# terminusdb-labs/parallel-hnsw

Hardware: AMD Instinct MI355X
Metric: queries/sec at recall@10≥0.95 on 1M×768 f32 (higher is better)
Workload: dtype f32

## Files before the change

### parallel_hnsw_amd/csrc/api.hip

```cpp
#include <hip/hip_runtime.h>

#include <algorithm>
#include <atomic>
#include <cmath>
#include <cstdarg>
#include <cstdio>
#include <cstring>
#include <new>
#include <stdexcept>
#include <vector>

#include "exact_slices.h"
#include "phnsw_internal.h"

static thread_local std::string g_err;

void ph_set_error(const char *fmt, ...) {
  char buf[1024];
  va_list ap;
  va_start(ap, fmt);
  vsnprintf(buf, sizeof(buf), fmt, ap);
  va_end(ap);
  g_err = buf;
}
// ... 763 lines not shown
    if (!rc && c.first_node + nq <= B.n_nodes) rc = ph_layer_range_order(B, c.first_node, (uint32_t)nq, &a.order);
    if (rc) return rc;
  }
  const bool split = (ph_store_f32(ix->store) || ph_store_converted(ix->store)) && !a.order && !knn_mode && !out_stride && !out_index && first_big < a.n_layers &&
                     nq >= two_launch_min() &&
                     !getenv("PHNSW_NO_LOCALITY");
  if (split) {
    g_two_launch_count++;
    rc = ph_workspace_order_ensure(ws, a.nq);
    for (uint32_t l = first_big; l < a.n_layers && !rc; l++)
      rc = ph_layer_anchor_pos(ix->store, mix->layers[l - 1]);
    if (rc) return rc;
    if (a.collect_k) {
      const size_t need = (size_t)nq * a.ef * 4u;
      if (ws.park_ids_bytes < need) {
        if (ws.park_ids) PH_HIP(hipFree(ws.park_ids));
        ws.park_ids = nullptr, ws.park_ids_bytes = 0;
        PH_HIP(hipMalloc(&ws.park_ids, need));
        ws.park_ids_bytes = need;
      }
      if (ws.park_d_bytes < need) {
        if (ws.park_d) PH_HIP(hipFree(ws.park_d));
        ws.park_d = nullptr, ws.park_d_bytes = 0;
        PH_HIP(hipMalloc(&ws.park_d, need));
        ws.park_d_bytes = need;
      }
      a.out_ids = ws.park_ids;
      a.out_d = ws.park_d;
    }
  }
  const uint32_t *table_pos = nullptr;
  const char *const table_order_env = getenv("PHNSW_TABLE_ORDER");
  if (T && !split && !a.order && !knn_mode && !out_stride && !out_index && !c.hint && !c.out_hit && !a.filter && !a.label_of && !a.attr_of && !a.pair_of &&
      !a.collect_k && nq >= PH_TABLE_ORDER_MIN && !getenv("PHNSW_NO_LOCALITY") && !(table_order_env && table_order_env[0] == '0')) {
    PhLayerHost &TL = mix->layers[T - 1];
    rc = ph_layer_anchor_pos(ix->store, TL);
    if (!rc && TL.pos) rc = ph_workspace_order_ensure(ws, a.nq);
    if (rc) return rc;
    table_pos = TL.pos;
  }
  rc = attach_probes(mix, c, a);
  if (rc) return rc;
  rc = ph_search_begin(ws, stream);
  if (rc) return rc;
  bool kept_table = false;
  if (c.hint && T && !split) {
    rc = ph_build_table_prepare(mix, ws, a, *c.hint, T, stream, &kept_table);
    if (rc) return rc;
  }
  const uint64_t tmax = (T && !kept_table) ? ph_tiny_max_positions(ix, a.n_layers, a.ef) : 0;
  const uint64_t chunk = (tmax && nq > tmax) ? tmax : nq;
  for (uint64_t c0 = 0; c0 < nq; c0 += chunk) {
    PhSearchArgs b = a;
    const uint64_t cnt = std::min<uint64_t>(chunk, nq - c0);
    const bool last_chunk = c0 + cnt == nq;
    b.nq = (uint32_t)cnt;
    if (b.order) {
      b.order += c0;
    } else if (c0) {
      const uint32_t ostride = out_stride ? out_stride : b.ef;
      if (b.queries) b.queries += c0 * c.ldq;
      if (b.qids) b.qids += c0;
      if (b.exclude) b.exclude += c0;
      if (b.filter) b.filter += c0 * b.filter_stride;
      if (b.label_want) b.label_want += c0;
      if (b.range_lo) b.range_lo += c0, b.range_hi += c0;
      if (b.pair_want) b.pair_want += c0;
      if (b.pair_lo) b.pair_lo += c0, b.pair_hi += c0;
      if (b.set_first) b.set_first += c0;
      if (b.out_ids) b.out_ids += c0 * ostride, b.out_d += c0 * ostride;
      if (b.collect_k) b.collect_ids += c0 * b.collect_k, b.collect_d += c0 * b.collect_k;
      b.out_len += c0;
      if (b.out_stats) b.out_stats += 2 * c0;
      b.status += c0;
      if (b.out_hit) b.out_hit += c0;
      b.first_node += (uint32_t)c0;
    }
    ws.n_chunks = (uint32_t)(c0 / chunk) + 1;
    PH_HIP(hipEventRecord(ws.evc, stream));
    if (c0) PH_HIP(hipMemsetAsync(ws.dtotals, 0, sizeof(unsigned long long) * 3 * PH_MAX_DISPATCH, stream));
    if (!kept_table) {
      rc = ph_tiny_prepare(ix, ws, b, T, stream);
      if (!rc && table_pos && b.tiny_layers == T) {
        rc = ph_tiny_table_order(ws, b, table_pos, ix->store->n_anchors, stream);
        if (!rc && b.table_by_query) g_table_order_count++;
      }
      if (rc) return rc;
    }
    ws.d_tiny = b.tiny_layers != 0;
    PH_HIP(hipEventRecord(ws.evd[0], stream));
    if (!split) {
      b.launch_totals = ws.dtotals;
      b.launch_tab = ws.dtotals + 2 * PH_MAX_DISPATCH;
      rc = ph_search_launch(ix, ws, b, stream, last_chunk);
      if (rc) return rc;
      PH_HIP(hipEventRecord(ws.evd[1], stream));
      ws.n_dispatch = 1;
      ws.d_lo[0] = knn_mode ? b.n_layers - 1 : 0;
      ws.d_hi[0] = b.n_layers;
      continue;
    }
    const uint32_t Td = b.tiny_layers;
    const bool dense_first = Td && Td < b.n_layers && b.nq >= PH_DENSE_SPLIT_MIN && !getenv("PHNSW_NO_DENSE_SPLIT");
    if (dense_first) b.dense_flag = ws.tiny_member + b.tiny_n;
    uint32_t di = 0;
    uint32_t *const out_hit_final = b.out_hit;
    const uint32_t first_hi = dense_first ? Td : first_big;
    for (uint32_t lo = 0, hi = first_hi; lo < b.n_layers; lo = hi, hi = (lo == Td && dense_first && first_big > Td) ? first_big : hi + 1) {
      PhSearchArgs p = b;
      const bool last = hi == b.n_layers;
      p.layer_lo = lo;
      p.layer_hi = hi;
      if (lo) p.tiny_layers = 0;
      if (dense_first) {
        p.dense_only = lo == 0 ? 1u : 0u;
        p.after_dense = lo == Td ? Td : 0u;
      }
      if (!last && p.collect_k) {
        p.collect_k = p.collect_flags = 0u;
        p.filter = nullptr, p.filter_stride = 0u;
        p.label_of = p.label_want = nullptr;
      }
      p.order = lo ? ws.oorder : nullptr;
      p.out_hit = last ? out_hit_final : nullptr;
      p.out_key = last ? nullptr : ws.okey;
      p.key_pos = last ? nullptr : ix->layers[hi - 1].pos;
      p.launch_totals = ws.dtotals + 2 * di;
      p.launch_tab = ws.dtotals + 2 * PH_MAX_DISPATCH + di;
      rc = ph_search_launch(ix, ws, p, stream, last && last_chunk);
      if (!rc && !last) rc = ph_workspace_order_sort(ws, b.nq, stream);
      if (rc) return rc;
      PH_HIP(hipEventRecord(ws.evd[1 + di], stream));
      ws.d_lo[di] = lo;
      ws.d_hi[di] = hi;
      ws.n_dispatch = ++di;
    }
  }
  return 0;
}

static int check_device_call(const char *call, const phnsw_index *ix, const PhSearchCall &c) {
  int rc = ph_check_sp(ix, c.sp);
  if (rc) return rc;
  if ((!c.queries && !c.qids) || !c.out_ids || !c.out_d || !c.out_len || !c.status || c.nq > 0xFFFFFFFFull ||
      (c.queries && (c.ldq < ix->store->ld || (c.ldq % 4) || ((uintptr_t)c.queries % 16)))) {
    ph_set_error("%s: invalid argument (queries need ldq >= store ld, multiple of 4, 16-byte base)", call);
    return PHNSW_E_INVALID;
  }
  return 0;
}

static PhSearchCall device_call(const float *queries_dev, uint32_t ldq, const uint32_t *qids_dev, uint64_t nq,
                                const phnsw_search_params *sp, uint32_t upto_layers, const uint32_t *exclude_dev,
                                uint32_t *out_ids_dev, float *out_d_dev, uint32_t *out_len_dev, uint32_t *out_stats_dev,
                                uint32_t *status_dev, void *stream) {
  PhSearchCall c = {};
  c.queries = queries_dev, c.ldq = ldq, c.qids = qids_dev, c.exclude = exclude_dev, c.nq = nq;
  c.sp = sp, c.upto = upto_layers;
  c.out_ids = out_ids_dev, c.out_d = out_d_dev, c.out_len = out_len_dev, c.status = status_dev;
  c.out_stats = out_stats_dev;
  c.stream = (hipStream_t)stream;
  return c;
}

extern "C" int phnsw_search_batch_device(const phnsw_index *ix, const float *queries_dev, uint32_t ldq,
                                         const uint32_t *qids_dev, uint64_t nq, const phnsw_search_params *sp,
                                         uint32_t upto_layers, const uint32_t *exclude_dev, uint32_t *out_ids_dev,
// ... 591 lines not shown
```

### parallel_hnsw_amd/csrc/bruteforce.hip

```cpp
#include <hip/hip_runtime.h>

#include <algorithm>
#include <cstring>
#include <vector>

#include "phnsw_device.h"

typedef float f32x16 __attribute__((ext_vector_type(16)));

#define BF_TM 128
#define BF_TN 128
#define BF_TK 32
#define BF_LD 132

__global__ __launch_bounds__(256) void ph_gemm_nt_mfma_kernel(const float *__restrict__ Q, uint32_t ldq, uint32_t nq,
                                                              const float *__restrict__ B, uint32_t ldb, uint32_t nb,
                                                              uint32_t K, float *__restrict__ C, uint64_t ldc) {
  __shared__ float Qs[BF_TK][BF_LD];
  __shared__ float Bs[BF_TK][BF_LD];
  const uint32_t t = threadIdx.x, lane = t & 63, w = t >> 6;
  const uint32_t wm = w >> 1, wn = w & 1;
  const uint32_t q0 = blockIdx.y * BF_TM, b0 = blockIdx.x * BF_TN;
  f32x16 acc[2][2];
#pragma unroll
// ... 273 lines not shown
}

__global__ __launch_bounds__(256) void ph_anchor_mean_kernel(const float *__restrict__ rows, uint64_t row_stride, uint32_t ld,
                                                             const uint32_t *__restrict__ start,
                                                             const uint32_t *__restrict__ members, uint32_t A,
                                                             const float *__restrict__ old, float *__restrict__ out) {
  __shared__ float wsum[4];
  const uint32_t a = blockIdx.x, t = threadIdx.x;
  if (a >= A) return;
  const uint32_t first = start[a], cnt = start[a + 1u] - first;
  float ss = 0.f;
  for (uint32_t j = t; j < ld; j += 256u) {
    float acc = 0.f;
    for (uint32_t i = 0; i < cnt; i++) acc += rows[(uint64_t)members[first + i] * row_stride + j];
    out[(uint64_t)a * ld + j] = acc;
    ss += acc * acc;
  }
#pragma unroll
  for (int sft = 32; sft >= 1; sft >>= 1) ss += __shfl_xor(ss, sft);
  if ((t & 63u) == 0) wsum[t >> 6] = ss;
  __syncthreads();
  const float norm = sqrtf(((wsum[0] + wsum[1]) + wsum[2]) + wsum[3]);
  const bool keep = !(norm > 0.f) || !(norm < PH_FMAX);
  for (uint32_t j = t; j < ld; j += 256u)
    out[(uint64_t)a * ld + j] = keep ? old[(uint64_t)a * ld + j] : out[(uint64_t)a * ld + j] / norm;
}

#define PH_CELL_SAMPLE 262144u

static int ph_refine_anchors(const phnsw_store *s, uint32_t A, const float *raw, float *refined) {
  const uint32_t ld = s->ld, m = (uint32_t)std::min<uint64_t>(s->n, PH_CELL_SAMPLE);
  const uint64_t step = s->n / m;
  const uint32_t QC = 65536;
  float *samp = nullptr, *scores = nullptr;
  uint32_t *cell = nullptr, *start = nullptr, *members = nullptr, *ids = nullptr;
  const float *base = s->rows;
  uint64_t row_stride = step * ld;
  int rc = 0;
  hipError_t e = hipMalloc(&scores, (size_t)std::min(QC, m) * A * 4);
  if (e == hipSuccess) e = hipMalloc(&cell, (size_t)m * 4);
  if (e == hipSuccess) e = hipMalloc(&start, ((size_t)A + 1u) * 4);
  if (e == hipSuccess) e = hipMalloc(&members, (size_t)m * 4);
  if (e == hipSuccess && (ph_store_converted(s) || row_stride > 0xFFFFFFFCull)) {
    std::vector<uint32_t> h(m);
    for (uint32_t i = 0; i < m; i++) h[i] = (uint32_t)(i * step);
    e = hipMalloc(&samp, (size_t)m * ld * 4);
    if (e == hipSuccess) e = hipMalloc(&ids, (size_t)m * 4);
    if (e == hipSuccess) e = hipMemcpy(ids, h.data(), (size_t)m * 4, hipMemcpyHostToDevice);
    if (e == hipSuccess) {
      if (ph_store_converted(s))
        rc = ph_converted_gather_rows(s, ids, 0, m, samp);
      else
        hipLaunchKernelGGL(ph_gather_rows_f32_kernel, dim3((m + 3) / 4), dim3(256), 0, 0, s->rows, ld, ids, 1u, m, samp);
    }
    base = samp;
    row_stride = ld;
  }
  if (e == hipSuccess && !rc) {
    for (uint32_t at = 0; at < m; at += QC) {
      const uint32_t cnt = std::min(QC, m - at);
      dim3 grid((A + BF_TN - 1) / BF_TN, (cnt + BF_TM - 1) / BF_TM);
      hipLaunchKernelGGL(ph_gemm_nt_mfma_kernel, grid, dim3(256), 0, 0, base + (uint64_t)at * row_stride, (uint32_t)row_stride,
                         cnt, raw, ld, A, ld, scores, (uint64_t)A);
      hipLaunchKernelGGL(ph_argmax_rows_kernel, dim3(std::min<uint32_t>(cnt, 256u * 16u)), dim3(64), 0, 0, scores, (uint64_t)A,
                         A, cnt, cell + at);
    }
    rc = ph_cell_order_device(cell, m, A, start, members, 0);
    if (!rc) {
      hipLaunchKernelGGL(ph_anchor_mean_kernel, dim3(A), dim3(256), 0, 0, base, row_stride, ld, start, members, A, raw, refined);
      e = hipGetLastError();
      if (e == hipSuccess) e = hipDeviceSynchronize();
    }
  }
  if (e != hipSuccess) rc = ph_hip_fail(e, "store cells (anchor means)", __FILE__, __LINE__);
  if (samp) hipFree(samp);
  if (ids) hipFree(ids);
  if (scores) hipFree(scores);
  if (cell) hipFree(cell);
  if (start) hipFree(start);
  if (members) hipFree(members);
  return rc;
}

static int ph_store_anchors(phnsw_store *s) {
  if (s->anchors) return 0;
  uint32_t amax = 4096u;
  if (const char *e = getenv("PHNSW_ANCHORS")) amax = atoi(e) >= 64 ? (uint32_t)atoi(e) : amax;
  const uint32_t A = (uint32_t)std::min<uint64_t>(amax, std::max<uint64_t>(s->n / 16u, 1u)), ld = s->ld;
  const uint64_t stride = s->n / A;
  const char *const cells_env = getenv("PHNSW_CELLS");
  const bool cells_raw = cells_env && !strcmp(cells_env, "raw");
  float *anchors = nullptr, *gram = nullptr;
  uint32_t *rank = nullptr, *ids = nullptr;
  std::vector<uint32_t> h(A);
  for (uint32_t a = 0; a < A; a++) h[a] = (uint32_t)(a * stride);
  hipError_t e = hipMalloc(&anchors, (size_t)A * ld * 4);
  if (e == hipSuccess) e = hipMalloc(&gram, (size_t)A * A * 4);
  if (e == hipSuccess) e = hipMalloc(&rank, (size_t)A * 4);
  if (e == hipSuccess) e = hipMalloc(&ids, (size_t)A * 4);
  if (e == hipSuccess) e = hipMemcpy(ids, h.data(), (size_t)A * 4, hipMemcpyHostToDevice);
  if (e == hipSuccess) {
    if (ph_store_converted(s))
      (void)ph_converted_gather_rows(s, ids, 0, A, anchors);
    else
      hipLaunchKernelGGL(ph_gather_rows_f32_kernel, dim3((A + 3) / 4), dim3(256), 0, 0, s->rows, ld, ids, 1u, A, anchors);
    if (!cells_raw) {
      float *refined = nullptr;
      e = hipMalloc(&refined, (size_t)A * ld * 4);
      if (e == hipSuccess && ph_refine_anchors(s, A, anchors, refined)) e = hipErrorUnknown;
      if (e == hipSuccess) std::swap(anchors, refined);
      if (refined) hipFree(refined);
    }
  }
  if (e == hipSuccess) {
    dim3 grid((A + BF_TN - 1) / BF_TN, (A + BF_TM - 1) / BF_TM);
    hipLaunchKernelGGL(ph_gemm_nt_mfma_kernel, grid, dim3(256), 0, 0, anchors, ld, A, anchors, ld, A, ld, gram, (uint64_t)A);
    hipLaunchKernelGGL(ph_anchor_chain_kernel, dim3(1), dim3(1024), (A + 32) * 4, 0, gram, A, rank);
    e = hipGetLastError();
    if (e == hipSuccess) e = hipDeviceSynchronize();
  }
  if (gram) hipFree(gram);
  if (ids) hipFree(ids);
  if (e != hipSuccess) {
    if (anchors) hipFree(anchors);
    if (rank) hipFree(rank);
    return ph_hip_fail(e, "store cells (anchors)", __FILE__, __LINE__);
  }
  s->anchors = anchors;
  s->anchor_rank = rank;
  s->n_anchors = A;
  s->cells_raw = cells_raw;
  return 0;
}

void ph_store_anchors_free(phnsw_store *s) {
  if (s->anchors) hipFree(s->anchors);
  if (s->anchor_rank) hipFree(s->anchor_rank);
  s->anchors = nullptr;
  s->anchor_rank = nullptr;
}

bool ph_layer_wants_cells(const phnsw_store *s, uint32_t n_nodes) {
  return n_nodes >= PH_POS_MIN && (ph_store_f32(s) || ph_store_converted(s)) && s->n >= 65536 && s->metric != PHNSW_METRIC_L2 && !getenv("PHNSW_NO_LOCALITY");
}

int ph_layer_cells_range(const phnsw_store *cs, const PhLayerHost &L, uint32_t first, uint32_t count, uint32_t *out_pos) {
  phnsw_store *s = const_cast<phnsw_store *>(cs);
  if (count == 0) return 0;
  int rc = ph_store_anchors(s);
  if (rc) return rc;
  const uint32_t A = s->n_anchors, ld = s->ld;
  const uint32_t QC = 65536;
  float *qrows = nullptr, *scores = nullptr;
  hipError_t e = hipMalloc(&scores, (size_t)std::min(QC, count) * A * 4);
  if (e == hipSuccess && (!L.identity || ph_store_converted(s))) e = hipMalloc(&qrows, (size_t)std::min(QC, count) * ld * 4);
  if (e == hipSuccess) {
    for (uint32_t at = 0; at < count; at += QC) {
      const uint32_t cnt = std::min(QC, count - at);
      const float *Q = ph_store_f32(s) ? s->rows + (uint64_t)(first + at) * ld : nullptr;
      if (ph_store_converted(s)) {
        (void)ph_converted_gather_rows(s, L.identity ? nullptr : L.nodes + first + at, first + at, cnt, qrows);
        Q = qrows;
      } else if (!L.identity) {
        hipLaunchKernelGGL(ph_gather_rows_f32_kernel, dim3((cnt + 3) / 4), dim3(256), 0, 0, s->rows, ld, L.nodes + first + at,
                           1u, cnt, qrows);
        Q = qrows;
      }
      dim3 grid((A + BF_TN - 1) / BF_TN, (cnt + BF_TM - 1) / BF_TM);
      hipLaunchKernelGGL(ph_gemm_nt_mfma_kernel, grid, dim3(256), 0, 0, Q, ld, cnt, s->anchors, ld, A,
                         s->cells_raw ? std::min<uint32_t>(ld, 256u) : ld, scores, (uint64_t)A);
      hipLaunchKernelGGL(ph_argmax_rows_kernel, dim3(std::min<uint32_t>(cnt, 256u * 16u)), dim3(64), 0, 0, scores,
                         (uint64_t)A, A, cnt, out_pos + at);
    }
    hipLaunchKernelGGL(ph_rank_of_cell_kernel, dim3((count + 255) / 256), dim3(256), 0, 0, out_pos, count, s->anchor_rank);
    e = hipGetLastError();
    if (e == hipSuccess) e = hipDeviceSynchronize();
  }
  if (e != hipSuccess) rc = ph_hip_fail(e, "layer cells (anchor GEMM)", __FILE__, __LINE__);
  if (qrows) hipFree(qrows);
  if (scores) hipFree(scores);
  return rc;
}

int ph_layer_anchor_pos(const phnsw_store *cs, PhLayerHost &L) {
  const uint32_t n = L.n_nodes;
  if (L.pos || !ph_layer_wants_cells(cs, n)) return 0;
  hipError_t e = hipMalloc(&L.pos, (size_t)n * 4);
  if (e != hipSuccess) return ph_hip_fail(e, "layer cells", __FILE__, __LINE__);
  int rc = ph_layer_cells_range(cs, L, 0, n, L.pos);
  if (rc) {
    hipFree(L.pos);
    L.pos = nullptr;
  }
  return rc;
}

extern "C" int phnsw_debug_store_cells(phnsw_store *s, float *anchors_out, uint32_t *rank_out, uint32_t *n_anchors_out) try {
  if (!s || !n_anchors_out || !(ph_store_f32(s) || ph_store_converted(s)) || s->n < 16 || s->metric == PHNSW_METRIC_L2) {
    ph_set_error("phnsw_debug_store_cells: need an f32, f16 or i8 store with a dot-product metric");
    return PHNSW_E_INVALID;
  }
  PH_HIP(hipSetDevice(s->device));
  if (int rc = ph_store_anchors(s)) return rc;
  *n_anchors_out = s->n_anchors;
  if (anchors_out) PH_HIP(hipMemcpy(anchors_out, s->anchors, (size_t)s->n_anchors * s->ld * 4, hipMemcpyDeviceToHost));
  if (rank_out) PH_HIP(hipMemcpy(rank_out, s->anchor_rank, (size_t)s->n_anchors * 4, hipMemcpyDeviceToHost));
  return 0;
} catch (...) { return ph_caught(); }

extern "C" int phnsw_debug_layer_cells(phnsw_index *ix, uint32_t lft, uint32_t *pos_out) try {
  if (!ix || !pos_out || lft >= ix->layers.size()) {
    ph_set_error("phnsw_debug_layer_cells: invalid argument");
    return PHNSW_E_INVALID;
  }
  PH_HIP(hipSetDevice(ix->store->device));
  PhLayerHost &L = ix->layers[lft];
  if (int rc = ph_layer_anchor_pos(ix->store, L)) return rc;
  if (!L.pos) {
    ph_set_error("phnsw_debug_layer_cells: layer %u carries no cells", lft);
    return PHNSW_E_UNSUPPORTED;
  }
// ... 39 lines not shown
```

### parallel_hnsw_amd/csrc/phnsw_internal.h

```cpp
#pragma once
#include <hip/hip_runtime.h>
#include <stdint.h>
#include <stdlib.h>

#include <mutex>
#include <string>
#include <vector>

#include "../../include/phnsw.h"

#define PH_EMPTY32 0xFFFFFFFFu
#define PH_FMAX 3.4028234663852886e38f
#define PH_MAX_LAYERS 24
#define PH_WAVE 64
#define PH_MAX_DISPATCH 24
#define PH_DENSE_SPLIT_MIN 2048u
#define PH_TINY_MAX_NODES 8192u
#define PH_TINY_LDS_NODES 1024u
#define PH_TINY_MAX_LAYERS 8

void ph_set_error(const char *fmt, ...);
int ph_caught() noexcept;
int ph_hip_fail(hipError_t e, const char *what, const char *file, int line);
#define PH_HIP(x)                                                       \
  do {                                                                  \
    hipError_t e__ = (x);                                               \
    if (e__ != hipSuccess) return ph_hip_fail(e__, #x, __FILE__, __LINE__); \
  } while (0)

struct PhLayerDev {
  uint32_t n_nodes;
  uint32_t W;
  const uint32_t *nodes;
  const uint32_t *neighbors;
  const uint32_t *vec2node;
};

struct PhLayerHost {
  uint32_t n_nodes = 0, W = 0;
  uint32_t *nodes = nullptr;
  uint32_t *neighbors = nullptr;
  float *nbr_dist = nullptr;
  uint64_t links_epoch = 0;
  uint32_t *vec2node = nullptr;
  bool identity = false;
  uint32_t *recall_q = nullptr;
  uint32_t recall_n = 0;
  uint32_t *pos = nullptr;
  uint32_t *ord = nullptr;
  uint32_t ord_first = 0, ord_count = 0;
};

enum PhRowKind : int {
  PH_ROWS_F32 = 0,
  PH_ROWS_F16,
  PH_ROWS_I8,
  PH_ROWS_PQ,
  PH_ROWS_PQ_SHARED,
  PH_ROWS_I8Q,
};
static inline bool ph_rows_converted(int kind) { return kind == PH_ROWS_F16 || kind == PH_ROWS_I8 || kind == PH_ROWS_I8Q; }
static inline bool ph_rows_i8_layout(int kind) { return kind == PH_ROWS_I8 || kind == PH_ROWS_I8Q; }
static inline const char *ph_rows_name(int kind) {
  static const char *const names[] = {"f32", "f16", "i8", "product-quantised", "shared-codebook product-quantised", "i8q"};
  return names[kind];
}
static inline int ph_chunk_count(uint32_t nv4) { return nv4 <= 64 ? 1 : (nv4 <= 192 ? 3 : (nv4 <= 384 ? 6 : 0)); }
int ph_dim_unsupported(uint32_t dim);
struct PhRows {
  const void *base;
  uint32_t stride;
  int kind;
};

struct PhDistArgs {
  PhRows rows;
  uint32_t ld, nv4;
  int metric;
  const uint8_t *codes;
  const uint16_t *codes16;
  const float *codebook;
  uint32_t m, ksub, dsub;
  uint32_t table_f16;
};

struct phnsw_store {
  int device = 0;
  int kind = PH_ROWS_F32;
  float *rows = nullptr;
  uint8_t *codes = nullptr;
  uint16_t *codes16 = nullptr;
  phnsw_store *centroid_store = nullptr;
  phnsw_index *centroid_index = nullptr;
  phnsw_search_params quantized_search = {0, 0, 0};
  float *codebook = nullptr;
  uint32_t pq_m = 0, pq_ksub = 0, pq_dsub = 0;
  uint32_t pq_table_f16 = 0;
  void *packed = nullptr;
  uint32_t packed_stride = 0;
  float *anchors = nullptr;
  uint32_t *anchor_rank = nullptr;
  uint32_t n_anchors = 0;
  bool cells_raw = false;
  bool owns_rows = true;
  uint64_t n = 0;
  uint32_t dim = 0, ld = 0;
  int metric = 0;
  int refcount = 1;
};

struct PhTinyPrepKey {
  bool valid = false;
  uint64_t nodes_epoch = 0;
  uint32_t T = 0, tn = 0;
  const void *nodes[PH_TINY_MAX_LAYERS] = {}, *nbrs[PH_TINY_MAX_LAYERS] = {}, *vec2node = nullptr;
  uint32_t n[PH_TINY_MAX_LAYERS] = {}, W[PH_TINY_MAX_LAYERS] = {};
  uint64_t links[PH_TINY_MAX_LAYERS] = {};
};
struct PhTinyPackKey {
  bool valid = false;
  uint64_t nodes_epoch = 0;
  const void *vecs = nullptr, *tnodes = nullptr;
  uint32_t ld = 0, tn = 0, nv = 0;
};

struct PhWorkspace {
  uint32_t *visited = nullptr;
  uint64_t visited_words = 0;
  uint2 *ovf = nullptr;
  uint32_t ovf_cap = 0;
  uint32_t n_slots = 0;
  uint32_t *counter = nullptr;
  hipEvent_t ev0 = nullptr, ev1 = nullptr;
  hipEvent_t evc = nullptr;
  bool timed = false;
  void *pq_tables = nullptr;
  size_t pq_tables_bytes = 0;
  uint32_t *okey = nullptr, *okey_sorted = nullptr, *oiota = nullptr, *oorder = nullptr;
  void *sort_tmp = nullptr;
  size_t sort_tmp_bytes = 0;
  uint32_t order_cap = 0;
  uint32_t *ocell = nullptr;
  uint32_t ocell_cap = 0;
  float *tiny_d = nullptr;
  size_t tiny_d_bytes = 0;
  uint32_t *tiny_nbr = nullptr;
  size_t tiny_nbr_bytes = 0;
  uint32_t *tiny_member = nullptr;
  size_t tiny_member_bytes = 0;
  float4 *tiny_pq = nullptr, *tiny_pn = nullptr;
  size_t tiny_pq_bytes = 0, tiny_pn_bytes = 0;
  PhTinyPrepKey tiny_prep_key;
  PhTinyPackKey tiny_pack_key;
  int tiny_table_g = 0;
  uint32_t tiny_last_npos = 0, tiny_last_tn = 0, tiny_last_stride = 0;
  uint2 *dense_ovf = nullptr;
  size_t dense_ovf_bytes = 0;
  uint32_t *ovf_s = nullptr;
  size_t ovf_s_cap = 0;
  uint32_t *park_ids = nullptr;
  float *park_d = nullptr;
  size_t park_ids_bytes = 0, park_d_bytes = 0;
  hipEvent_t evd[PH_MAX_DISPATCH + 1] = {};
  unsigned long long *dtotals = nullptr;
  uint32_t n_dispatch = 0;
  uint32_t n_chunks = 0;
  int cus = 0;
  uint32_t d_lo[PH_MAX_DISPATCH] = {}, d_hi[PH_MAX_DISPATCH] = {};
  bool d_tiny = false;
};

struct PhBuildTable {
  float *D = nullptr;
  size_t bytes = 0;
  size_t cap = 0;
  const uint32_t *qnodes = nullptr, *tnodes = nullptr;
  uint32_t qn = 0, tn = 0, T = 0, stride = 0;
  uint32_t lo_alloc = 0, hi_alloc = 0, lo = 0, hi = 0;
  uint64_t epoch = 0;
};
struct PhRowHint {
  const uint32_t *qnodes;
  uint32_t qn;
// ... 297 lines not shown
  uint32_t *out_len, *status;
  hipStream_t stream;
  const uint32_t *list;
};
int ph_labeled_device(const phnsw_index *ix, const phnsw_labels *lb, const PhLabeledCall &c);
struct PhLabelsetCall {
  PhLabeledCall c;
  const uint32_t *want_first, *want_values;
  uint64_t nwant, batch_nq;
};
int ph_labelset_device(const phnsw_index *ix, const phnsw_labels *lb, const PhLabelsetCall &sc);
int ph_labels_count_set(const phnsw_labels *lb, const uint32_t *want_first_dev, const uint32_t *want_values_dev, uint64_t nq,
                        uint64_t nwant, uint32_t *out_count_dev, uint32_t *owner_scratch, hipStream_t stream);
int ph_labels_fresh(const phnsw_index *ix, const phnsw_labels *lb, const char *call);
int ph_labeled_check(const phnsw_index *ix, const phnsw_labels *lb, uint64_t k, const char *call);
const uint32_t *ph_labels_column(const phnsw_labels *lb);
int ph_labels_count(const phnsw_labels *lb, const uint32_t *want_dev, uint64_t nq, uint32_t *out_count_dev, hipStream_t stream);
struct PhRangedCall {
  const float *queries;
  uint32_t ldq;
  const uint32_t *qids, *exclude, *lo, *hi;
  uint64_t nq;
  uint32_t k;
  uint32_t *out_ids;
  float *out_d;
  uint32_t *out_len, *status;
  hipStream_t stream;
  const uint32_t *list;
};
int ph_ranged_device(const phnsw_index *ix, const phnsw_attr *at, const PhRangedCall &c);
int ph_attr_fresh(const phnsw_index *ix, const phnsw_attr *at, const char *call);
int ph_ranged_check(const phnsw_index *ix, const phnsw_attr *at, uint64_t k, const char *call);
const uint32_t *ph_attr_column(const phnsw_attr *at);
int ph_attr_count(const phnsw_attr *at, const uint32_t *lo_dev, const uint32_t *hi_dev, uint64_t nq, uint32_t *out_count_dev,
                  hipStream_t stream);
struct PhLabelRangedCall {
  const float *queries;
  uint32_t ldq;
  const uint32_t *qids, *exclude, *want, *lo, *hi;
  uint64_t nq;
  uint32_t k;
  uint32_t *out_ids;
  float *out_d;
  uint32_t *out_len, *status;
  hipStream_t stream;
  const uint32_t *list;
};
int ph_label_ranged_device(const phnsw_index *ix, const phnsw_label_attr *h, const PhLabelRangedCall &c);
int ph_label_attr_fresh(const phnsw_index *ix, const phnsw_label_attr *h, const char *call);
int ph_label_ranged_check(const phnsw_index *ix, const phnsw_label_attr *h, uint64_t k, const char *call);
const uint64_t *ph_label_attr_column(const phnsw_label_attr *h);
int ph_label_attr_count(const phnsw_label_attr *h, const uint32_t *want_dev, const uint32_t *lo_dev, const uint32_t *hi_dev,
                        uint64_t nq, uint32_t *out_count_dev, hipStream_t stream);
struct PhLabelsetRangedCall {
  PhLabelRangedCall c;
  const uint32_t *want_first, *want_values;
  uint64_t nwant, batch_nq;
};
int ph_labelset_ranged_device(const phnsw_index *ix, const phnsw_label_attr *h, const PhLabelsetRangedCall &sc);
int ph_label_attr_count_set(const phnsw_label_attr *h, const uint32_t *want_first_dev, const uint32_t *want_values_dev,
                            const uint32_t *lo_dev, const uint32_t *hi_dev, uint64_t nq, uint64_t nwant, uint32_t *out_count_dev,
                            uint32_t *owner_scratch, hipStream_t stream);
void ph_auto_free(phnsw_index *ix);
void ph_dense_free(phnsw_index *ix);
int ph_dense_check(const phnsw_index *ix, uint64_t k, const char *call);
void ph_grouped_free(phnsw_index *ix);
int ph_exact_check(const phnsw_index *ix, uint64_t k, const char *call);
#define PH_ORDER_MIN 16384u
#define PH_POS_MIN 256u
#define PH_TABLE_ORDER_MIN 2048u
#define PH_SPLIT_BYTES (4ull << 20)
static inline bool ph_layer_own_launch(uint64_t n_nodes, uint32_t row_bytes) {
  const char *e = getenv("PHNSW_SPLIT_BYTES");
  const uint64_t limit = (e && atoll(e) > 0) ? (uint64_t)atoll(e) : (uint64_t)PH_SPLIT_BYTES;
  return n_nodes * (uint64_t)row_bytes > limit;
}
int ph_layer_anchor_pos(const phnsw_store *s, PhLayerHost &L);
bool ph_layer_wants_cells(const phnsw_store *s, uint32_t n_nodes);
int ph_layer_cells_range(const phnsw_store *s, const PhLayerHost &L, uint32_t first, uint32_t count, uint32_t *out_pos);
void ph_store_anchors_free(phnsw_store *s);
int ph_order_by_keys_device(const uint32_t *keys, uint32_t n, uint32_t *order_out, hipStream_t st);
int ph_layer_range_order(PhLayerHost &L, uint32_t first, uint32_t count, const uint32_t **out);
int ph_cell_order_device(const uint32_t *keys, uint32_t n, uint32_t bins, uint32_t *start, uint32_t *order_out, hipStream_t st);
int ph_tiny_table_order(PhWorkspace &ws, PhSearchArgs &b, const uint32_t *pos, uint32_t bins, hipStream_t stream);

static inline bool ph_store_converted(const phnsw_store *s) { return ph_rows_converted(s->kind); }
static inline bool ph_store_f32(const phnsw_store *s) { return s->kind == PH_ROWS_F32; }
static inline bool ph_store_pq(const phnsw_store *s) { return s->kind == PH_ROWS_PQ; }
static inline bool ph_store_pq_shared(const phnsw_store *s) { return s->kind == PH_ROWS_PQ_SHARED; }
int ph_converted_gather_rows(const phnsw_store *s, const uint32_t *ids_dev, uint32_t first, uint32_t cnt, float *out_dev);
int ph_converted_store_read(const phnsw_store *s, uint64_t first, uint64_t count, float *out);

int ph_tiny_prepare(const phnsw_index *ix, PhWorkspace &ws, PhSearchArgs &a, uint32_t max_layers, hipStream_t stream);
int ph_build_table_prepare(phnsw_index *ix, PhWorkspace &ws, PhSearchArgs &a, const PhRowHint &h, uint32_t T,
                           hipStream_t stream, bool *used);
void ph_build_table_free(phnsw_index *ix);
size_t ph_tiny_lds_bytes(const PhSearchArgs &a);
bool ph_tiny_matrix_cores(const phnsw_index *ix);
uint32_t ph_tiny_layer_count(const phnsw_index *ix, uint32_t n_layers, uint32_t ef);
uint64_t ph_tiny_max_positions(const phnsw_index *ix, uint32_t n_layers, uint32_t ef);
void ph_tiny_free(PhWorkspace &ws);
int ph_tiny_table_chunk(const phnsw_index *ix, PhWorkspace &ws, const float *queries, uint32_t ldq, const uint32_t *qids,
                        const uint32_t *order, uint32_t npos, const uint32_t *tnodes, uint32_t tn, float *D, hipStream_t stream,
                        bool *kept);

int ph_search_begin(PhWorkspace &ws, hipStream_t stream);
int ph_search_launch(const phnsw_index *ix, PhWorkspace &ws, PhSearchArgs &a, hipStream_t stream, bool mark_end = true);
int ph_search_launch_big(const phnsw_index *ix, PhSearchArgs &a, uint32_t grid, hipStream_t stream);
int ph_workspace_order_ensure(PhWorkspace &ws, uint32_t nq);
int ph_workspace_order_sort(PhWorkspace &ws, uint32_t nq, hipStream_t stream);
void ph_workspace_order_free(PhWorkspace &ws);
#define PH_TWO_LAUNCH_MIN 32768u
int ph_workspace_ensure(const phnsw_index *ix, PhWorkspace &ws, uint32_t ef, uint32_t ovf_cap);
void ph_workspace_free(PhWorkspace &ws);
size_t ph_tiny_beside_lds(const phnsw_index *ix, const PhSearchArgs &a);
static inline PhRows ph_store_rows(const phnsw_store *s) {
  PhRows r;
  r.base = ph_store_converted(s) ? (const void *)s->packed : (const void *)s->rows;
  r.stride = ph_store_converted(s) ? s->packed_stride : s->ld * 4u;
  r.kind = s->kind;
  return r;
}
static inline PhDistArgs ph_dist_args(const phnsw_store *s) {
  PhDistArgs d;
  d.rows = ph_store_rows(s);
  d.ld = s->ld;
  d.nv4 = s->ld / 4;
  d.metric = s->metric;
  d.codes = s->codes;
  d.codes16 = s->codes16;
  d.codebook = s->codebook;
  d.m = s->pq_m;
  d.ksub = s->pq_ksub;
  d.dsub = s->pq_dsub;
  d.table_f16 = s->pq_table_f16;
  return d;
}
static inline uint32_t ph_row_bytes(const phnsw_store *s) { return ph_store_rows(s).stride; }
static inline int ph_search_only_unsupported(const phnsw_store *s, const char *call) {
  if (!s || !ph_store_converted(s)) return 0;
  ph_set_error("%s: not supported on an %s store or an index over one (search-only; use the f32 store)", call,
               ph_rows_name(s->kind));
  return PHNSW_E_UNSUPPORTED;
}
static inline bool ph_pq_global_tables() {
  const char *e = getenv("PHNSW_PQ_TABLE");
  return !(e && e[0] == 'l');
}
static inline size_t ph_pq_lds_bytes(const phnsw_store *s) {
  return ph_store_pq(s) ? (size_t)s->pq_m * s->pq_ksub * (s->pq_table_f16 == 2 ? 1 : (s->pq_table_f16 ? 2 : 4)) : 0;
}

void ph_comm_range(const phnsw_comm *comm, uint32_t r, uint64_t n, uint64_t *chunk, uint64_t *first, uint64_t *count);
int ph_comm_all_gather_device(const phnsw_comm *comm, const void *send_dev, void *recv_dev, uint64_t bytes);

int ph_synth_rows(float *rows_dev, uint64_t first, uint64_t count, uint32_t dim, uint32_t ld,
                  uint64_t seed, int normalize, hipStream_t s);
int ph_synth_clustered_rows(float *rows_dev, uint64_t first, uint64_t count, uint32_t dim, uint32_t ld, uint64_t seed,
                            uint32_t n_clusters, float noise, hipStream_t s);
int ph_distance_batch(const phnsw_store *st, const float *q_dev, uint32_t query_id, const uint32_t *ids_dev,
                      uint32_t k, float *out_dev, hipStream_t s);
int ph_fill_u32(uint32_t *p, uint32_t v, uint64_t n, hipStream_t s);
int ph_take_launch(const uint32_t *ids, const float *d, uint32_t ef, uint32_t k, uint64_t n, uint64_t *ids64, float *dk,
                   hipStream_t s);
int ph_scatter_vec2node(const uint32_t *nodes, uint32_t n, uint32_t *vec2node, hipStream_t s);
int ph_count_nan(const float *rows, uint64_t n_floats, uint32_t *out_count_dev, hipStream_t s);

// ... 37 lines not shown
```

### parallel_hnsw_amd/csrc/tiny.hip

```cpp
#include <hip/hip_runtime.h>

#include <algorithm>
#include <cstdlib>
#include <cstring>

#include "phnsw_device.h"

struct PhTinyPrepArgs {
  PhLayerDev layers[PH_TINY_MAX_LAYERS];
  uint32_t T, tiny_n;
  uint32_t off[PH_TINY_MAX_LAYERS];
  uint32_t *nbr;
  uint32_t *member;
};

__global__ void ph_tiny_prep_kernel(PhTinyPrepArgs p) {
  const uint32_t l = blockIdx.y;
  const PhLayerDev L = p.layers[l], TL = p.layers[p.T - 1];
  for (uint32_t i = blockIdx.x * blockDim.x + threadIdx.x; i < L.n_nodes; i += gridDim.x * blockDim.x) {
    const uint32_t vid = L.nodes[i];
    const uint32_t t = TL.vec2node ? TL.vec2node[vid] : vid;
    if (t >= p.tiny_n) {
      p.member[p.tiny_n] = 1u;
      continue;
// ... 761 lines not shown
  }
  const int mode = table_beside_mode();
  bool beside = mode == 1;
  if (mode == 2) {
    const PhWorkspace &other = &ws == &ix->ws[0] ? ix->ws[1] : ix->ws[0];
    if ((&ws == &ix->ws[0] || &ws == &ix->ws[1]) && other.timed && other.ev1) {
      beside = hipEventQuery(other.ev1) == hipErrorNotReady;
      (void)hipGetLastError();
    }
  }
  bool prep_kept = false, pack_kept = false;
  int rc = tiny_prep_graph(ix, ws, a, T, tn, stream, &prep_kept);
  if (rc) return rc < 0 ? rc : 0;
  rc = tiny_table(ix, ws, a.dist, a.queries, a.ldq, a.qids, a.order, npos, a.layers[T - 1].nodes, tn, stride, ws.tiny_d, stream,
                  beside ? 1 : 2, &pack_kept);
  if (rc) return rc < 0 ? rc : 0;
  if (getenv("PHNSW_VERBOSE")) {
    if (ws.tiny_table_g)
      fprintf(stderr, "[phnsw] dense table: %u positions x %u nodes on the matrix cores, G = %d (%s), graph %s, node operand %s\n",
              npos, tn, ws.tiny_table_g, beside ? "beside the other workspace's launch" : "alone",
              prep_kept ? "kept" : "prepared", pack_kept ? "kept" : "packed");
    else
      fprintf(stderr, "[phnsw] dense table: %u positions x %u nodes on the vector units, graph %s\n", npos, tn,
              prep_kept ? "kept" : "prepared");
  }
  ws.tiny_last_npos = npos;
  ws.tiny_last_tn = tn;
  ws.tiny_last_stride = stride;
  a.tiny_layers = T;
  a.tiny_n = tn;
  a.tiny_lds_nodes = PH_TINY_LDS_NODES;
  a.tiny_stride = stride;
  a.tiny_d = ws.tiny_d;
  a.tiny_nbr = ws.tiny_nbr;
  a.tiny_member = ws.tiny_member;
  return 0;
}


__global__ __launch_bounds__(64) void ph_tiny_row_cell_kernel(const float *__restrict__ D, uint32_t stride, uint32_t tn,
                                                              uint32_t nq, const uint32_t *__restrict__ pos,
                                                              uint32_t *__restrict__ key) {
  const uint32_t lane = threadIdx.x;
  for (uint32_t q = blockIdx.x; q < nq; q += gridDim.x) {
    const float *row = D + (uint64_t)q * stride;
    uint64_t top[4] = {KEY_NONE, KEY_NONE, KEY_NONE, KEY_NONE};
    for (uint32_t t = lane; t < tn; t += 64) {
      uint64_t k = mkkey(row[t], t);
      if (k < top[3]) {
#pragma unroll
        for (int j = 0; j < 4; j++) {
          const uint64_t lo = k < top[j] ? k : top[j], hi = k < top[j] ? top[j] : k;
          top[j] = lo;
          k = hi;
        }
      }
    }
    uint32_t cell[4], n = 0;
#pragma unroll
    for (int r = 0; r < 4; r++) {
      uint64_t m = top[0];
#pragma unroll
      for (int s = 32; s >= 1; s >>= 1) {
        const uint64_t o = __shfl_xor(m, s);
        m = o < m ? o : m;
      }
      if (top[0] == m) top[0] = top[1], top[1] = top[2], top[2] = top[3], top[3] = KEY_NONE;
      const uint32_t t = (uint32_t)m & IDM;
      cell[r] = 0u;
      if (m != KEY_NONE && t < tn) cell[r] = pos[t], n = r + 1;
    }
    uint32_t best = 0, best_cnt = 0;
#pragma unroll
    for (int i = 0; i < 4; i++) {
      uint32_t cnt = 0;
#pragma unroll
      for (int j = 0; j < 4; j++) cnt += ((uint32_t)j < n && cell[j] == cell[i]) ? 1u : 0u;
      if ((uint32_t)i < n && cnt > best_cnt) best = cell[i], best_cnt = cnt;
    }
    if (lane == 0) key[q] = best;
  }
}

int ph_tiny_table_order(PhWorkspace &ws, PhSearchArgs &b, const uint32_t *pos, uint32_t bins, hipStream_t stream) {
  if (!b.tiny_layers || b.tiny_rows || !pos || !bins || ws.order_cap < b.nq) return 0;
  if (ws.ocell_cap < bins) {
    if (ws.ocell) PH_HIP(hipFree(ws.ocell));
    ws.ocell = nullptr, ws.ocell_cap = 0;
    PH_HIP(hipMalloc(&ws.ocell, ((size_t)bins + 1u) * 4u));
    ws.ocell_cap = bins;
  }
  hipLaunchKernelGGL(ph_tiny_row_cell_kernel, dim3(std::min<uint32_t>(b.nq, 1u << 16)), dim3(64), 0, stream, b.tiny_d,
                     b.tiny_stride, b.tiny_n, b.nq, pos, ws.okey);
  int rc = ph_cell_order_device(ws.okey, b.nq, bins, ws.ocell, ws.oorder, stream);
  if (rc) return rc;
  b.order = ws.oorder;
  b.table_by_query = 1u;
  return 0;
}


void ph_build_table_free(phnsw_index *ix) {
  for (PhBuildTable &b : ix->bt)
    if (b.D) ph_timed_free(b.D);
  ix->bt.clear();
  for (auto &sp : ix->bt_spare) ph_timed_free(sp.first);
  ix->bt_spare.clear();
}
static void build_table_drop(phnsw_index *ix, PhBuildTable &b) {
  if (b.D) ix->bt_spare.emplace_back(b.D, b.cap);
  b.D = nullptr;
  b.bytes = b.cap = 0;
  b.lo = b.hi = b.lo_alloc = b.hi_alloc = 0;
}
static void build_table_recycle(phnsw_index *ix) {
  for (PhBuildTable &b : ix->bt) build_table_drop(ix, b);
  ix->bt.clear();
}
static float *build_table_buffer(phnsw_index *ix, size_t bytes, size_t *cap) {
  int best = -1;
  for (size_t i = 0; i < ix->bt_spare.size(); i++)
    if (ix->bt_spare[i].second >= bytes && ix->bt_spare[i].second <= 2 * bytes &&
        (best < 0 || ix->bt_spare[i].second < ix->bt_spare[(size_t)best].second))
      best = (int)i;
  if (best >= 0) {
    float *p = ix->bt_spare[(size_t)best].first;
    *cap = ix->bt_spare[(size_t)best].second;
    ix->bt_spare.erase(ix->bt_spare.begin() + best);
    return p;
  }
  size_t mfree = 0, mtotal = 0;
  if (hipMemGetInfo(&mfree, &mtotal) != hipSuccess) return nullptr;
  size_t want = bytes + bytes / 16;
  if (want + (8ull << 30) > mfree) {
    for (auto &sp : ix->bt_spare) ph_timed_free(sp.first);
    ix->bt_spare.clear();
    if (hipMemGetInfo(&mfree, &mtotal) != hipSuccess) return nullptr;
    want = bytes;
  }
  if (want + (8ull << 30) > mfree || bytes > mtotal / 2) return nullptr;
  float *p = nullptr;
  if (ph_timed_malloc((void **)&p, want) != hipSuccess) {
    (void)hipGetLastError();
    return nullptr;
  }
  *cap = want;
  return p;
}

static uint32_t build_table_min() {
  if (const char *e = getenv("PHNSW_BUILD_TABLE_MIN"))
    if (atoi(e) > 0) return (uint32_t)atoi(e);
  return 1024u;
}

int ph_build_table_prepare(phnsw_index *ix, PhWorkspace &ws, PhSearchArgs &a, const PhRowHint &h, uint32_t T,
                           hipStream_t stream, bool *used) {
  *used = false;
  a.tiny_rows = 0;
  if (!ix->bt_enabled || !T || !a.qids || a.queries || a.knn_mode || a.layer_lo || getenv("PHNSW_NO_BUILD_TABLE")) return 0;
  const uint32_t tn = ix->layers[T - 1].n_nodes, stride = tiny_stride_of(tn);
  const uint32_t *tnodes = a.layers[T - 1].nodes;
  if (tn < build_table_min() || h.qn == 0) return 0;
  if (!ix->bt.empty() && ix->bt[0].epoch != ix->nodes_epoch) build_table_recycle(ix);
  PhBuildTable *found = nullptr;
  for (PhBuildTable &b : ix->bt)
    if (b.qnodes == h.qnodes && b.qn == h.qn) found = &b;
  if (!found) {
    if (ix->bt.size() >= PH_MAX_LAYERS) return 0;
    ix->bt.emplace_back();
    found = &ix->bt.back();
    found->epoch = ix->nodes_epoch;
    found->qnodes = h.qnodes;
    found->qn = h.qn;
  }
  PhBuildTable &B = *found;
  const uint32_t need_lo = h.contiguous ? h.first : 0u, need_hi = h.contiguous ? h.first + h.count : h.qn;
  if (need_hi > h.qn || need_lo >= need_hi) return 0;
  const bool same = B.D && B.tnodes == tnodes && B.tn == tn && B.T == T;
  if (B.D && !same) build_table_drop(ix, B);
  if (!h.contiguous && !(B.D && B.lo <= need_lo && B.hi >= need_hi)) return 0;
  if (!B.D || need_lo < B.lo_alloc || need_hi > B.hi_alloc) {
// ... 58 lines not shown
```

Baseline: 1.235 million.

## Refine query cell ordering by scoring neighboring anchor cells against the query

Query ordering for table search used to key each query by the most common cell among its top few tiny-table entries. The new path takes the T nearest tiny-table entries, expands each to the ±R neighboring cells in anchor rank order, and scores those anchors against the query directly, keying the query by the best one. Anchors are stored again in rank order so that neighboring cells sit next to each other in memory. The goal is better query locality and cache reuse during the main search, at the cost of an extra per-query kernel that reads anchor vectors. A debug entry point for checking the keys is also added.

```diff
diff --git a/parallel_hnsw_amd/csrc/api.hip b/parallel_hnsw_amd/csrc/api.hip
--- a/parallel_hnsw_amd/csrc/api.hip
+++ b/parallel_hnsw_amd/csrc/api.hip
@@ -869,7 +869,7 @@
     if (!kept_table) {
       rc = ph_tiny_prepare(ix, ws, b, T, stream);
       if (!rc && table_pos && b.tiny_layers == T) {
-        rc = ph_tiny_table_order(ws, b, table_pos, ix->store->n_anchors, stream);
+        rc = ph_tiny_table_order(ix->store, ws, b, table_pos, stream);
         if (!rc && b.table_by_query) g_table_order_count++;
       }
       if (rc) return rc;
diff --git a/parallel_hnsw_amd/csrc/bruteforce.hip b/parallel_hnsw_amd/csrc/bruteforce.hip
--- a/parallel_hnsw_amd/csrc/bruteforce.hip
+++ b/parallel_hnsw_amd/csrc/bruteforce.hip
@@ -379,7 +379,14 @@
   return rc;
 }
 
-static int ph_store_anchors(phnsw_store *s) {
+__global__ void ph_anchor_by_rank_kernel(const float *__restrict__ anchors, const uint32_t *__restrict__ rank, uint32_t A,
+                                         uint32_t ld, float *__restrict__ by_rank) {
+  const uint32_t a = blockIdx.x;
+  if (a >= A || rank[a] >= A) return;
+  for (uint32_t j = threadIdx.x; j < ld; j += blockDim.x) by_rank[(uint64_t)rank[a] * ld + j] = anchors[(uint64_t)a * ld + j];
+}
+
+int ph_store_anchors(phnsw_store *s) {
   if (s->anchors) return 0;
   uint32_t amax = 4096u;
   if (const char *e = getenv("PHNSW_ANCHORS")) amax = atoi(e) >= 64 ? (uint32_t)atoi(e) : amax;
@@ -387,13 +394,14 @@
   const uint64_t stride = s->n / A;
   const char *const cells_env = getenv("PHNSW_CELLS");
   const bool cells_raw = cells_env && !strcmp(cells_env, "raw");
-  float *anchors = nullptr, *gram = nullptr;
+  float *anchors = nullptr, *gram = nullptr, *ranked = nullptr;
   uint32_t *rank = nullptr, *ids = nullptr;
   std::vector<uint32_t> h(A);
   for (uint32_t a = 0; a < A; a++) h[a] = (uint32_t)(a * stride);
   hipError_t e = hipMalloc(&anchors, (size_t)A * ld * 4);
   if (e == hipSuccess) e = hipMalloc(&gram, (size_t)A * A * 4);
   if (e == hipSuccess) e = hipMalloc(&rank, (size_t)A * 4);
+  if (e == hipSuccess) e = hipMalloc(&ranked, (size_t)A * ld * 4);
   if (e == hipSuccess) e = hipMalloc(&ids, (size_t)A * 4);
   if (e == hipSuccess) e = hipMemcpy(ids, h.data(), (size_t)A * 4, hipMemcpyHostToDevice);
   if (e == hipSuccess) {
@@ -413,6 +421,7 @@
     dim3 grid((A + BF_TN - 1) / BF_TN, (A + BF_TM - 1) / BF_TM);
     hipLaunchKernelGGL(ph_gemm_nt_mfma_kernel, grid, dim3(256), 0, 0, anchors, ld, A, anchors, ld, A, ld, gram, (uint64_t)A);
     hipLaunchKernelGGL(ph_anchor_chain_kernel, dim3(1), dim3(1024), (A + 32) * 4, 0, gram, A, rank);
+    hipLaunchKernelGGL(ph_anchor_by_rank_kernel, dim3(A), dim3(256), 0, 0, anchors, rank, A, ld, ranked);
     e = hipGetLastError();
     if (e == hipSuccess) e = hipDeviceSynchronize();
   }
@@ -420,10 +429,12 @@
   if (ids) hipFree(ids);
   if (e != hipSuccess) {
     if (anchors) hipFree(anchors);
+    if (ranked) hipFree(ranked);
     if (rank) hipFree(rank);
     return ph_hip_fail(e, "store cells (anchors)", __FILE__, __LINE__);
   }
   s->anchors = anchors;
+  s->anchors_ranked = ranked;
   s->anchor_rank = rank;
   s->n_anchors = A;
   s->cells_raw = cells_raw;
@@ -432,8 +443,10 @@
 
 void ph_store_anchors_free(phnsw_store *s) {
   if (s->anchors) hipFree(s->anchors);
+  if (s->anchors_ranked) hipFree(s->anchors_ranked);
   if (s->anchor_rank) hipFree(s->anchor_rank);
   s->anchors = nullptr;
+  s->anchors_ranked = nullptr;
   s->anchor_rank = nullptr;
 }
 
diff --git a/parallel_hnsw_amd/csrc/phnsw_internal.h b/parallel_hnsw_amd/csrc/phnsw_internal.h
--- a/parallel_hnsw_amd/csrc/phnsw_internal.h
+++ b/parallel_hnsw_amd/csrc/phnsw_internal.h
@@ -99,6 +99,7 @@
   void *packed = nullptr;
   uint32_t packed_stride = 0;
   float *anchors = nullptr;
+  float *anchors_ranked = nullptr;
   uint32_t *anchor_rank = nullptr;
   uint32_t n_anchors = 0;
   bool cells_raw = false;
@@ -562,7 +563,10 @@
 int ph_order_by_keys_device(const uint32_t *keys, uint32_t n, uint32_t *order_out, hipStream_t st);
 int ph_layer_range_order(PhLayerHost &L, uint32_t first, uint32_t count, const uint32_t **out);
 int ph_cell_order_device(const uint32_t *keys, uint32_t n, uint32_t bins, uint32_t *start, uint32_t *order_out, hipStream_t st);
-int ph_tiny_table_order(PhWorkspace &ws, PhSearchArgs &b, const uint32_t *pos, uint32_t bins, hipStream_t stream);
+#define PH_ORDER_REFINE_T 6u
+#define PH_ORDER_REFINE_R 1u
+int ph_tiny_table_order(const phnsw_store *s, PhWorkspace &ws, PhSearchArgs &b, const uint32_t *pos, hipStream_t stream);
+int ph_store_anchors(phnsw_store *s);
 
 static inline bool ph_store_converted(const phnsw_store *s) { return ph_rows_converted(s->kind); }
 static inline bool ph_store_f32(const phnsw_store *s) { return s->kind == PH_ROWS_F32; }
diff --git a/parallel_hnsw_amd/csrc/tiny.hip b/parallel_hnsw_amd/csrc/tiny.hip
--- a/parallel_hnsw_amd/csrc/tiny.hip
+++ b/parallel_hnsw_amd/csrc/tiny.hip
@@ -867,7 +867,159 @@
   }
 }
 
-int ph_tiny_table_order(PhWorkspace &ws, PhSearchArgs &b, const uint32_t *pos, uint32_t bins, hipStream_t stream) {
+struct PhRowCellRefineArgs {
+  const float *D;
+  uint32_t stride, tn, nq;
+  const uint32_t *pos;
+  PhDistArgs dist;
+  const float *queries;
+  uint32_t ldq;
+  const uint32_t *qids;
+  const float *anchors;
+  uint32_t bins, ld, nv4;
+  uint32_t T, R;
+  uint32_t *key;
+};
+
+__device__ __forceinline__ uint64_t wave_min_key(uint64_t k) {
+  const uint32_t hi = wave_min_u32((uint32_t)(k >> 32));
+  const uint32_t lo = wave_min_u32((uint32_t)(k >> 32) == hi ? (uint32_t)k : 0xFFFFFFFFu);
+  return ((uint64_t)hi << 32) | lo;
+}
+
+#define PH_ORDER_REFINE_TMAX 16u
+template <int NV, class Rw>
+__global__ __launch_bounds__(64) void ph_tiny_row_cell_refine_kernel(PhRowCellRefineArgs a) {
+  const uint32_t lane = threadIdx.x, W = 2u * a.R + 1u;
+  const uint32_t r_of = lane / W, j_of = lane % W;
+  DistRows<NV, 1, Rw> qd;
+  for (uint32_t q = blockIdx.x; q < a.nq; q += gridDim.x) {
+    if (a.queries)
+      qd.prepare_raw(a.dist, a.queries + (uint64_t)q * a.ldq, nullptr, lane);
+    else
+      qd.prepare_stored(a.dist, a.qids[q], nullptr, lane);
+    const float *row = a.D + (uint64_t)q * a.stride;
+    uint64_t mine = KEY_NONE;
+    uint64_t last = KEY_NONE;
+    for (uint32_t t0 = 0; t0 < a.tn; t0 += 256u) {
+      float v[4];
+#pragma unroll
+      for (int u = 0; u < 4; u++) v[u] = t0 + 64u * u + lane < a.tn ? row[t0 + 64u * u + lane] : 0.f;
+#pragma unroll
+      for (int u = 0; u < 4; u++) {
+        const uint32_t t = t0 + 64u * u + lane;
+        const uint32_t f = fkey(v[u]);
+        uint64_t in = __ballot(t < a.tn && mkkey(v[u], t) < last);
+        while (in) {
+          const uint32_t src = (uint32_t)__builtin_ctzll(in);
+          in &= in - 1u;
+          const uint64_t k = ((uint64_t)rl32(f, (int)src) << 32) | (t0 + 64u * u + src);
+          if (k >= last) continue;
+          const uint32_t at = (uint32_t)__popcll(__ballot(lane < a.T && mine < k));
+          const uint32_t lo = (uint32_t)__builtin_amdgcn_update_dpp(0, (int)(uint32_t)mine, 0x111, 0xF, 0xF, false);
+          const uint32_t hi = (uint32_t)__builtin_amdgcn_update_dpp(0, (int)(uint32_t)(mine >> 32), 0x111, 0xF, 0xF, false);
+          if (lane == at) mine = k;
+          else if (lane > at) mine = ((uint64_t)hi << 32) | lo;
+          last = rl64(mine, (int)(a.T - 1u));
+        }
+      }
+    }
+    const uint32_t n = (uint32_t)__popcll(__ballot(lane < a.T && mine != KEY_NONE));
+    const uint32_t near_t = (uint32_t)mine & IDM;
+    const uint32_t t = __shfl(near_t, (int)min(r_of, 63u));
+    const bool slot = r_of < n && t < a.tn;
+    const uint32_t base = slot ? min(a.pos[t], a.bins - 1u) : 0u;
+    const int64_t c0 = (int64_t)base + (int64_t)j_of - (int64_t)a.R;
+    const bool valid = slot && c0 >= 0 && c0 < (int64_t)a.bins;
+    const uint32_t cell = valid ? (uint32_t)c0 : 0u;
+    bool dup = false;
+    for (uint32_t r = 0; r + 1u < n; r++) {
+      const uint32_t b = rl32(base, (int)(r * W));
+      if (r < r_of && cell + a.R >= b && cell <= b + a.R) dup = true;
+    }
+    uint64_t left = __ballot(valid && !dup);
+    float best = 0.f;
+    uint32_t best_cell = PH_EMPTY32;
+    while (left) {
+      uint32_t c[4], m = 0;
+#pragma unroll
+      for (int j = 0; j < 4; j++) {
+        c[j] = 0u;
+        if (left) {
+          c[j] = rl32(cell, __builtin_ctzll(left));
+          left &= left - 1u;
+          m = j + 1;
+        }
+      }
+      float acc[4] = {0.f, 0.f, 0.f, 0.f};
+#pragma unroll
+      for (int k = 0; k < NV; k++) {
+        const uint32_t ch = lane + 64u * k;
+        if (ch < a.nv4) {
+          float4 x[4];
+#pragma unroll
+          for (int j = 0; j < 4; j++) x[j] = ((const float4 *)(a.anchors + (uint64_t)c[j] * a.ld))[ch];
+#pragma unroll
+          for (int j = 0; j < 4; j++) {
+            acc[j] = fmaf(x[j].x, qd.qv[k].x, acc[j]);
+            acc[j] = fmaf(x[j].y, qd.qv[k].y, acc[j]);
+            acc[j] = fmaf(x[j].z, qd.qv[k].z, acc[j]);
+            acc[j] = fmaf(x[j].w, qd.qv[k].w, acc[j]);
+          }
+        }
+      }
+      const uint32_t s = __float_as_uint(wave_sum4(acc[0], acc[1], acc[2], acc[3]));
+      const float sc[4] = {__uint_as_float(rl32(s, 0)), __uint_as_float(rl32(s, 32)), __uint_as_float(rl32(s, 16)),
+                           __uint_as_float(rl32(s, 48))};
+#pragma unroll
+      for (int j = 0; j < 4; j++)
+        if ((uint32_t)j < m && (best_cell == PH_EMPTY32 || sc[j] > best || (sc[j] == best && c[j] < best_cell)))
+          best = sc[j], best_cell = c[j];
+    }
+    if (lane == 0) a.key[q] = best_cell == PH_EMPTY32 ? 0u : best_cell;
+  }
+}
+
+template <class Rw>
+static void row_cell_refine(const PhRowCellRefineArgs &a, hipStream_t stream) {
+  const dim3 grid(std::min<uint32_t>(a.nq, 1u << 16));
+  if (a.nv4 <= 192u)
+    hipLaunchKernelGGL((ph_tiny_row_cell_refine_kernel<3, Rw>), grid, dim3(64), 0, stream, a);
+  else
+    hipLaunchKernelGGL((ph_tiny_row_cell_refine_kernel<6, Rw>), grid, dim3(64), 0, stream, a);
+}
+
+static void table_keys(const phnsw_store *s, const PhDistArgs &dist, const float *D, uint32_t stride, uint32_t tn, uint32_t nq,
+                       const uint32_t *pos, const float *queries, uint32_t ldq, const uint32_t *qids, uint32_t *key,
+                       hipStream_t stream) {
+  const char *const refine_env = getenv("PHNSW_TABLE_ORDER_REFINE");
+  const bool rows = dist.rows.kind == PH_ROWS_F32 || ph_rows_converted(dist.rows.kind);
+  if ((refine_env && refine_env[0] == '0') || !s->anchors_ranked || !rows || (!queries && !qids) || s->ld > 1536u) {
+    hipLaunchKernelGGL(ph_tiny_row_cell_kernel, dim3(std::min<uint32_t>(nq, 1u << 16)), dim3(64), 0, stream, D, stride, tn, nq,
+                       pos, key);
+    return;
+  }
+  uint32_t T = PH_ORDER_REFINE_T, R = PH_ORDER_REFINE_R;
+  if (const char *e = getenv("PHNSW_TABLE_ORDER_T")) T = (uint32_t)std::max(1, atoi(e));
+  if (const char *e = getenv("PHNSW_TABLE_ORDER_R")) R = (uint32_t)std::max(0, atoi(e));
+  T = std::min(T, PH_ORDER_REFINE_TMAX);
+  R = std::min(R, (64u / T - 1u) / 2u);
+  PhRowCellRefineArgs a;
+  a.D = D, a.stride = stride, a.tn = tn, a.nq = nq, a.pos = pos, a.dist = dist;
+  a.queries = queries, a.ldq = ldq, a.qids = qids;
+  a.anchors = s->anchors_ranked, a.bins = s->n_anchors, a.ld = s->ld;
+  a.nv4 = (s->cells_raw ? std::min<uint32_t>(s->ld, 256u) : s->ld) / 4u;
+  a.T = T, a.R = R, a.key = key;
+  switch (dist.rows.kind) {
+    case PH_ROWS_F16: row_cell_refine<RowF16>(a, stream); break;
+    case PH_ROWS_I8:
+    case PH_ROWS_I8Q: row_cell_refine<RowI8>(a, stream); break;
+    default: row_cell_refine<RowF32>(a, stream); break;
+  }
+}
+
+int ph_tiny_table_order(const phnsw_store *s, PhWorkspace &ws, PhSearchArgs &b, const uint32_t *pos, hipStream_t stream) {
+  const uint32_t bins = s->n_anchors;
   if (!b.tiny_layers || b.tiny_rows || !pos || !bins || ws.order_cap < b.nq) return 0;
   if (ws.ocell_cap < bins) {
     if (ws.ocell) PH_HIP(hipFree(ws.ocell));
@@ -875,14 +1027,49 @@
     PH_HIP(hipMalloc(&ws.ocell, ((size_t)bins + 1u) * 4u));
     ws.ocell_cap = bins;
   }
-  hipLaunchKernelGGL(ph_tiny_row_cell_kernel, dim3(std::min<uint32_t>(b.nq, 1u << 16)), dim3(64), 0, stream, b.tiny_d,
-                     b.tiny_stride, b.tiny_n, b.nq, pos, ws.okey);
+  table_keys(s, b.dist, b.tiny_d, b.tiny_stride, b.tiny_n, b.nq, pos, b.queries, b.ldq, b.qids, ws.okey, stream);
   int rc = ph_cell_order_device(ws.okey, b.nq, bins, ws.ocell, ws.oorder, stream);
   if (rc) return rc;
   b.order = ws.oorder;
   b.table_by_query = 1u;
   return 0;
 }
+
+extern "C" int phnsw_debug_table_order_keys(phnsw_store *s, const float *D, uint32_t stride, uint32_t tn, uint32_t nq,
+                                            const uint32_t *pos, const float *queries, uint32_t ldq, uint32_t *keys_out) try {
+  if (!s || !D || !pos || !queries || !keys_out || nq == 0 || tn > stride || ldq < s->ld || (ldq & 3u) ||
+      !(ph_store_f32(s) || ph_store_converted(s)) || s->n < 16 || s->metric == PHNSW_METRIC_L2) {
+    ph_set_error("phnsw_debug_table_order_keys: invalid argument, or not an f32, f16 or i8 store with a dot-product metric");
+    return PHNSW_E_INVALID;
+  }
+  PH_HIP(hipSetDevice(s->device));
+  if (int rc = ph_store_anchors(s)) return rc;
+  for (uint32_t t = 0; t < tn; t++)
+    if (pos[t] >= s->n_anchors) {
+      ph_set_error("phnsw_debug_table_order_keys: pos[%u] = %u is no cell of %u", t, pos[t], s->n_anchors);
+      return PHNSW_E_INVALID;
+    }
+  float *d = nullptr, *qd = nullptr;
+  uint32_t *p = nullptr, *k = nullptr;
+  hipError_t e = ph_pool_alloc((void **)&d, std::max<size_t>((size_t)nq * stride * 4, 4));
+  if (e == hipSuccess) e = ph_pool_alloc((void **)&qd, (size_t)nq * ldq * 4);
+  if (e == hipSuccess) e = ph_pool_alloc((void **)&p, std::max<size_t>((size_t)tn * 4, 4));
+  if (e == hipSuccess) e = ph_pool_alloc((void **)&k, (size_t)nq * 4);
+  if (e == hipSuccess && stride) e = hipMemcpy(d, D, (size_t)nq * stride * 4, hipMemcpyHostToDevice);
+  if (e == hipSuccess) e = hipMemcpy(qd, queries, (size_t)nq * ldq * 4, hipMemcpyHostToDevice);
+  if (e == hipSuccess && tn) e = hipMemcpy(p, pos, (size_t)tn * 4, hipMemcpyHostToDevice);
+  if (e == hipSuccess) e = hipMemset(k, 0xFF, (size_t)nq * 4);
+  if (e == hipSuccess) {
+    table_keys(s, ph_dist_args(s), d, stride, tn, nq, p, qd, ldq, nullptr, k, 0);
+    e = hipGetLastError();
+  }
+  if (e == hipSuccess) e = hipMemcpy(keys_out, k, (size_t)nq * 4, hipMemcpyDeviceToHost);
+  if (d) ph_pool_free(d);
+  if (qd) ph_pool_free(qd);
+  if (p) ph_pool_free(p);
+  if (k) ph_pool_free(k);
+  return e == hipSuccess ? 0 : ph_hip_fail(e, "table order keys", __FILE__, __LINE__);
+} catch (...) { return ph_caught(); }
 
 
 void ph_build_table_free(phnsw_index *ix) {
```

After: 1.232 million, median of 3. No clear change (-0.3%).
